# IST-DASLab/torch_cgx

Measured on AMD Instinct MI355X. Metric: DDP samples/sec ResNet-50 4-bit, higher is better.
Workload: dtype bf16; 1 GPU; model=resnet50, global_batch=256, input=3x224x224, parallelism=dp1, backend=cgx, bits=4, bucket_size=1024, compression_active=False

## Files before the change

csrc/bindings.cc:

```cpp
#include <torch/extension.h>

#include <ATen/hip/impl/HIPStreamMasqueradingAsCUDA.h>
#include <torch/csrc/utils/pybind.h>

#include <ATen/hip/impl/HIPGuardImplMasqueradingAsCUDA.h>

#include <cstring>
#include <functional>
#include <thread>
#include <tuple>

#include "backend.h"
#include "bn_plan.h"
#include "collectives.h"
#include "reducer.h"

namespace cgx {
namespace {

void run_rank_threads(int ws, int dev,
                      const std::function<void(int, hipStream_t)>& body,
                      const std::function<void()>& abort) {
  std::vector<hipStream_t> qs(ws, nullptr);
  for (auto& s : qs)
// ... 506 lines not shown
  if (!bn_tensor_ok(dy)) dy = dy.contiguous(at::MemoryFormat::ChannelsLast);
  if (!bn_tensor_ok(dy)) dy = dy.clone(at::MemoryFormat::ChannelsLast);
  if (mask.has_value())
    TORCH_CHECK(mask->is_cuda() && mask->scalar_type() == at::kByte &&
                    mask->is_contiguous() && mask->numel() == x.numel() / 8,
                "bn_act_backward: mask must hold one bit per element");
  auto dx = at::empty(x.sizes(), x.options(), at::MemoryFormat::ChannelsLast);
  auto stats = x.options().dtype(at::kFloat);
  auto dgamma = at::empty({c}, stats), dbeta = at::empty({c}, stats);
  c10::optional<at::Tensor> didentity;
  if (has_identity)
    didentity = mask.has_value()
                    ? at::empty(x.sizes(), x.options(),
                                at::MemoryFormat::ChannelsLast)
                    : dy;
  auto part = bn_workspace(p, x);
  BnBackwardArgs a;
  a.dy = dy.data_ptr();
  a.x = x.data_ptr();
  a.mean = bn_channel_vec(mean, c, "mean");
  a.invstd = bn_channel_vec(invstd, c, "invstd");
  a.weight = bn_channel_vec(weight, c, "weight");
  a.mask = mask.has_value() ? mask->data_ptr<uint8_t>() : nullptr;
  a.dx = dx.data_ptr();
  a.didentity =
      has_identity && mask.has_value() ? didentity->data_ptr() : nullptr;
  a.dgamma = dgamma.data_ptr<float>();
  a.dbeta = dbeta.data_ptr<float>();
  a.part = part.data_ptr<float>();
  launch_bn_backward(
      p, a, c10::hip::getCurrentHIPStreamMasqueradingAsCUDA(
                x.device().index()).stream());
  return {dx, dgamma, dbeta, didentity};
}

py::dict py_bn_plan(int64_t rows, int64_t channels) {
  const BnPlan p = bn_plan(rows, channels);
  py::dict d;
  d["eligible"] = p.eligible;
  d["threads"] = kBnThreads;
  d["cgs"] = p.cgs;
  d["tile_cgs"] = p.tc;
  d["ctiles"] = p.ctiles;
  d["rows_per_iter"] = p.rln;
  d["splits"] = p.splits;
  d["grid"] = p.grid;
  d["rows_per_thread"] = p.rows_per_thread;
  d["partial_floats"] = p.partial_floats;
  return d;
}

at::Tensor py_bn_sweep_indices(int64_t rows, int64_t channels) {
  const BnPlan p = bn_plan(rows, channels);
  TORCH_CHECK(p.eligible, "bn_sweep_indices: shape is not eligible");
  auto out = at::full({(int64_t)p.grid * kBnThreads, p.rows_per_thread + 1},
                      -1, at::TensorOptions().dtype(at::kLong));
  int64_t* o = out.data_ptr<int64_t>();
  const int64_t width = p.rows_per_thread + 1;
  for (int wg = 0; wg < p.grid; wg++)
    for (int tid = 0; tid < kBnThreads; tid++) {
      const BnSweep sw = bn_sweep(p, wg, tid);
      int64_t k = 0;
      for (int64_t r = sw.row; r < p.rows; r += sw.stride, k++) {
        TORCH_CHECK(k < width, "bn_sweep_indices: run longer than planned");
        o[((int64_t)wg * kBnThreads + tid) * width + k] = bn_vec(p, r, sw.cg);
      }
// ... 146 lines not shown
  m.def("plan_bucket", &cgx::py_plan_bucket, py::arg("layer_numels"),
        py::arg("layer_cfgs"), py::arg("dtype"), py::arg("fusion_bytes"),
        py::arg("min_elems"), py::arg("fake_ratio") = 1.0,
        py::arg("dummy") = false,
        "Test seam: the bucket plan for layers laid out back to back from "
        "byte offset 0 -> (uncomp [(byte_off, count)], chunks [[(byte_off, "
        "numel, bits, bucket)]]).");
  m.def("plan_chunk", &cgx::py_plan_chunk, py::arg("views"), py::arg("dtype"),
        py::arg("ws"), py::arg("skip_incomplete") = false,
        "Test seam: the rank plan of one chunk [(byte_off, numel, bits, "
        "bucket)] -> (offs, szs, comp, rs [[(byte_off, n, bits, bucket, "
        "comp_off, skip_incomplete, fb_off)]]).");
  m.def("route_quantize", &cgx::py_route_quantize, py::arg("slices"),
        "Test seam: the launch router's quantize plan for "
        "[(in, out, fb, n, bits, bucket, skip_incomplete)] (pointers as "
        "ints) -> [(bits, kind, descs, cum, any_residual, max_gpl)].");
  m.def("route_dequantize", &cgx::py_route_dequantize, py::arg("slices"),
        py::arg("dtype"), py::arg("src_stride") = 0, py::arg("nsrc") = 1,
        py::arg("add") = false,
        "Test seam: the launch router's dequantize plan for "
        "[(in, out, n, bits, bucket, skip_incomplete)] -> "
        "[(bits, kind, descs, total_groups, any_residual)].");
  m.def("bn_act_forward", &cgx::py_bn_act_forward, py::arg("x"),
        py::arg("identity"), py::arg("weight"), py::arg("bias"),
        py::arg("running_mean"), py::arg("running_var"), py::arg("momentum"),
        py::arg("eps"), py::arg("relu"),
        "Training-mode BatchNorm2d of a channels_last bf16 tensor, fused with "
        "an optional residual add and ReLU -> (out, mean, invstd, mask | "
        "None); updates the running statistics in place.");
  m.def("bn_act_backward", &cgx::py_bn_act_backward, py::arg("dy"),
        py::arg("x"), py::arg("mean"), py::arg("invstd"), py::arg("weight"),
        py::arg("mask"), py::arg("has_identity"),
        "Backward of bn_act_forward -> (dx, dgamma, dbeta, didentity | None).");
  m.def("bn_eligible", &cgx::py_bn_eligible, py::arg("x"),
        "True where the fused BatchNorm kernels take `x`: CUDA, bf16, dense "
        "channels_last, and a shape bn_plan calls eligible.");
  m.def("bn_plan", &cgx::py_bn_plan, py::arg("rows"), py::arg("channels"),
        "Test seam: the launch geometry of the fused BatchNorm kernels for a "
        "[rows, channels] activation.");
  m.def("bn_sweep_indices", &cgx::py_bn_sweep_indices, py::arg("rows"),
        py::arg("channels"),
        "Test seam: [grid*threads, rows_per_thread+1] int64, the 16-byte "
        "vector indices every thread visits (-1: none).");
  m.def("bn_partial_offsets", &cgx::py_bn_partial_offsets, py::arg("rows"),
        py::arg("channels"), py::arg("wg"),
        "Test seam: the partial-buffer floats workgroup `wg` writes.");
  m.attr("FLAG_SKIP_INCOMPLETE") = cgx::kFlagSkipIncomplete;
  m.attr("FLAG_TAIL_ONLY") = cgx::kFlagTailOnly;
  m.attr("KIND_FAST") = (int)cgx::kFast;
  m.attr("KIND_GENERIC") = (int)cgx::kGeneric;
  m.attr("KIND_TWO_PASS") = (int)cgx::kTwoPass;
  m.attr("KIND_SUB") = (int)cgx::kSub;
}
```

csrc/bn_kernels.hip:

```cpp
#include <hip/hip_runtime.h>

#include "bn_plan.h"
#include "check.h"

namespace cgx {
namespace {

constexpr int kT = kBnThreads;

__device__ inline void unpack8(const uint4& v, float (&f)[8]) {
  f[0] = __uint_as_float(v.x << 16);
  f[1] = __uint_as_float(v.x & 0xffff0000u);
  f[2] = __uint_as_float(v.y << 16);
  f[3] = __uint_as_float(v.y & 0xffff0000u);
  f[4] = __uint_as_float(v.z << 16);
  f[5] = __uint_as_float(v.z & 0xffff0000u);
  f[6] = __uint_as_float(v.w << 16);
  f[7] = __uint_as_float(v.w & 0xffff0000u);
}

__device__ inline unsigned bf16_bits(float f) {
  const unsigned u = __float_as_uint(f);
  if ((u & 0x7fffffffu) > 0x7f800000u) return (u >> 16) | 0x40u;
  return (u + 0x7fffu + ((u >> 16) & 1u)) >> 16;
// ... 351 lines not shown
    scale[j] *= invstd[j];
    mg[j] *= inv_r;
    mgx[j] *= inv_r;
  }
  auto one = [&](const uint4& dyv, const uint4& xv, unsigned mbits, int64_t i) {
    float g[8], xf[8];
    unsigned gb[8], o[8];
    masked_dy<RELU>(dyv, mbits, g, gb);
    unpack8(xv, xf);
#pragma unroll
    for (int j = 0; j < 8; j++) {
      const float xhat = (xf[j] - mean[j]) * invstd[j];
      o[j] = bf16_bits(scale[j] * ((g[j] - mg[j]) - xhat * mgx[j]));
    }
    dx[i] = pack8(o);
    if (ADD) didentity[i] = pack8(gb);
  };
  int64_t r = sw.row;
  for (; r + sw.stride < p.rows; r += 2 * sw.stride) {
    const int64_t i0 = bn_vec(p, r, sw.cg);
    const int64_t i1 = bn_vec(p, r + sw.stride, sw.cg);
    const uint4 a0 = dy[i0], a1 = dy[i1];
    const uint4 b0 = x[i0], b1 = x[i1];
    const unsigned m0 = RELU ? mask[i0] : 0xffu, m1 = RELU ? mask[i1] : 0xffu;
    one(a0, b0, m0, i0);
    one(a1, b1, m1, i1);
  }
  if (r < p.rows) {
    const int64_t i0 = bn_vec(p, r, sw.cg);
    one(dy[i0], x[i0], RELU ? mask[i0] : 0xffu, i0);
  }
}

int fin_grid(const BnPlan& p) {
  return (p.channels + kBnFinChannels - 1) / kBnFinChannels;
}

}

void launch_bn_forward(const BnPlan& p, const BnForwardArgs& a,
                       hipStream_t stream) {
  float* pmean = a.part;
  float* pm2 = a.part + p.partial_floats;
  float* pcnt = a.part + 2 * p.partial_floats;
  const uint4* x = static_cast<const uint4*>(a.x);
  const uint4* idn = static_cast<const uint4*>(a.identity);
  uint4* out = static_cast<uint4*>(a.out);
  const dim3 grid(p.grid), block(kT);
  hipLaunchKernelGGL(bn_stats, grid, block, 0, stream, x, pmean, pm2, pcnt, p);
  hipLaunchKernelGGL(bn_stats_finalize, dim3(fin_grid(p)), block, 0, stream,
                     pmean, pm2, pcnt, a.mean, a.invstd, a.running_mean,
                     a.running_var, a.momentum, a.eps, p);
#define CGX_BN_APPLY(RELU, ADD)                                              \
  hipLaunchKernelGGL((bn_apply<RELU, ADD>), grid, block, 0, stream, x, idn,  \
                     a.mean, a.invstd, a.weight, a.bias, out, a.mask, p)
  if (a.relu && idn) CGX_BN_APPLY(true, true);
  else if (a.relu) CGX_BN_APPLY(true, false);
  else if (idn) CGX_BN_APPLY(false, true);
  else CGX_BN_APPLY(false, false);
#undef CGX_BN_APPLY
  CGX_HIP_CHECK(hipGetLastError());
}

void launch_bn_backward(const BnPlan& p, const BnBackwardArgs& a,
                        hipStream_t stream) {
  float* psg = a.part;
  float* psgx = a.part + p.partial_floats;
  const uint4* dy = static_cast<const uint4*>(a.dy);
  const uint4* x = static_cast<const uint4*>(a.x);
  uint4* dx = static_cast<uint4*>(a.dx);
  uint4* did = static_cast<uint4*>(a.didentity);
  const dim3 grid(p.grid), block(kT);
  if (a.mask)
    hipLaunchKernelGGL(bn_bwd_reduce<true>, grid, block, 0, stream, dy, x,
                       a.mask, a.mean, a.invstd, psg, psgx, p);
  else
    hipLaunchKernelGGL(bn_bwd_reduce<false>, grid, block, 0, stream, dy, x,
                       a.mask, a.mean, a.invstd, psg, psgx, p);
  hipLaunchKernelGGL(bn_bwd_finalize, dim3(fin_grid(p)), block, 0, stream, psg,
                     psgx, a.dbeta, a.dgamma, p);
#define CGX_BN_DX(RELU, ADD)                                                 \
  hipLaunchKernelGGL((bn_bwd_dx<RELU, ADD>), grid, block, 0, stream, dy, x,  \
                     a.mask, a.mean, a.invstd, a.weight, a.dbeta, a.dgamma,  \
                     dx, did, p)
  if (a.mask && did) CGX_BN_DX(true, true);
  else if (a.mask) CGX_BN_DX(true, false);
  else CGX_BN_DX(false, false);
#undef CGX_BN_DX
  CGX_HIP_CHECK(hipGetLastError());
}

}
```

csrc/bn_plan.cc:

```cpp
#include "bn_plan.h"

#include <algorithm>

namespace cgx {

BnPlan bn_plan(int64_t rows, int64_t channels) {
  BnPlan p;
  p.rows = rows;
  p.channels = (int)std::min<int64_t>(std::max<int64_t>(channels, 0), 1 << 30);
  const bool pow2 = channels > 0 && (channels & (channels - 1)) == 0;
  p.eligible = pow2 && channels >= 8 && channels <= 2048 && rows >= 2 &&
               rows <= kBnMaxRows;
  if (!p.eligible) return p;

  p.cgs = p.channels / 8;
  p.tc = std::min(p.cgs, kBnMaxTileCgs);
  p.ctiles = p.cgs / p.tc;
  p.rln = kBnThreads / p.tc;
  const int64_t row_blocks = (rows + p.rln - 1) / p.rln;
  int64_t splits = std::min<int64_t>(row_blocks,
                                     std::max(1, kBnTargetWgs / p.ctiles));
  splits = std::min(splits, std::max<int64_t>(1, rows / 80));
  p.splits = (int)splits;
  p.grid = p.ctiles * p.splits;
  p.rows_per_thread = (int)((row_blocks + splits - 1) / splits);
  p.partial_floats = (int64_t)p.splits * p.channels;
  return p;
}

}
```

csrc/bn_plan.h:

```cpp
#pragma once

#include <hip/hip_runtime.h>

#include <cstdint>

namespace cgx {

constexpr int kBnThreads = 256;
constexpr int kBnTargetWgs = 1024;
constexpr int kBnMaxTileCgs = 32;
constexpr int kBnFinChannels = 4;

struct BnPlan {
  int64_t rows = 0;
  int channels = 0;
  bool eligible = false;
  int cgs = 0;
  int tc = 0;
  int ctiles = 0;
  int rln = 0;
  int splits = 0;
  int grid = 0;
  int rows_per_thread = 0;
  int64_t partial_floats = 0;
// ... 29 lines not shown
  const void* x;
  const void* identity;
  const float* weight;
  const float* bias;
  float* running_mean;
  float* running_var;
  float momentum, eps;
  bool relu;
  void* out;
  float* mean;
  float* invstd;
  uint8_t* mask;
  float* part;
};
void launch_bn_forward(const BnPlan& p, const BnForwardArgs& a,
                       hipStream_t stream);

struct BnBackwardArgs {
  const void* dy;
  const void* x;
  const float* mean;
  const float* invstd;
  const float* weight;
  const uint8_t* mask;
  void* dx;
  void* didentity;
  float* dgamma;
  float* dbeta;
  float* part;
};
void launch_bn_backward(const BnPlan& p, const BnBackwardArgs& a,
                        hipStream_t stream);

}
```

torch_cgx_amd/models/resnet.py:

```python

from __future__ import annotations

import torch
import torch.nn as nn

from ..ops.fused_bn import bn_act


class Bottleneck(nn.Module):
    expansion = 4

    def __init__(self, inplanes: int, planes: int, stride: int = 1,
                 downsample: nn.Module = None):
        super().__init__()
        self.conv1 = nn.Conv2d(inplanes, planes, 1, bias=False)
        self.bn1 = nn.BatchNorm2d(planes)
        self.conv2 = nn.Conv2d(planes, planes, 3, stride=stride, padding=1,
                               bias=False)
        self.bn2 = nn.BatchNorm2d(planes)
        self.conv3 = nn.Conv2d(planes, planes * self.expansion, 1, bias=False)
        self.bn3 = nn.BatchNorm2d(planes * self.expansion)
        self.relu = nn.ReLU(inplace=True)
        self.downsample = downsample
        self.stride = stride

    def forward(self, x):
        identity = x
        out = bn_act(self.bn1, self.conv1(x))
        out = bn_act(self.bn2, self.conv2(out))
        out = self.conv3(out)
        if self.downsample is not None:
            identity = self.downsample(x)
        return bn_act(self.bn3, out, identity)


class ResNet(nn.Module):
    def __init__(self, layers, num_classes: int = 1000):
        super().__init__()
        self.inplanes = 64
        self.conv1 = nn.Conv2d(3, 64, 7, stride=2, padding=3, bias=False)
        self.bn1 = nn.BatchNorm2d(64)
        self.relu = nn.ReLU(inplace=True)
        self.maxpool = nn.MaxPool2d(3, stride=2, padding=1)
        self.layer1 = self._make_layer(64, layers[0])
        self.layer2 = self._make_layer(128, layers[1], stride=2)
        self.layer3 = self._make_layer(256, layers[2], stride=2)
        self.layer4 = self._make_layer(512, layers[3], stride=2)
        self.avgpool = nn.AdaptiveAvgPool2d(1)
        self.fc = nn.Linear(512 * Bottleneck.expansion, num_classes)
        for m in self.modules():
            if isinstance(m, nn.Conv2d):
                nn.init.kaiming_normal_(m.weight, mode="fan_out",
                                        nonlinearity="relu")
            elif isinstance(m, nn.BatchNorm2d):
                nn.init.constant_(m.weight, 1)
                nn.init.constant_(m.bias, 0)

    def _make_layer(self, planes: int, blocks: int, stride: int = 1):
        downsample = None
        if stride != 1 or self.inplanes != planes * Bottleneck.expansion:
            downsample = nn.Sequential(
                nn.Conv2d(self.inplanes, planes * Bottleneck.expansion, 1,
                          stride=stride, bias=False),
                nn.BatchNorm2d(planes * Bottleneck.expansion),
            )
        layers = [Bottleneck(self.inplanes, planes, stride, downsample)]
        self.inplanes = planes * Bottleneck.expansion
        for _ in range(1, blocks):
            layers.append(Bottleneck(self.inplanes, planes))
        return nn.Sequential(*layers)

    def forward(self, x):
        x = self.maxpool(bn_act(self.bn1, self.conv1(x)))
        x = self.layer4(self.layer3(self.layer2(self.layer1(x))))
        x = self.avgpool(x).flatten(1)
        return self.fc(x)


def resnet50(num_classes: int = 1000) -> ResNet:
    return ResNet([3, 4, 6, 3], num_classes)


def resnet18(num_classes: int = 1000) -> nn.Module:

    class BasicBlock(nn.Module):
        def __init__(self, inp, planes, stride=1, down=None):
            super().__init__()
            self.c1 = nn.Conv2d(inp, planes, 3, stride, 1, bias=False)
            self.b1 = nn.BatchNorm2d(planes)
            self.c2 = nn.Conv2d(planes, planes, 3, 1, 1, bias=False)
            self.b2 = nn.BatchNorm2d(planes)
            self.down = down

        def forward(self, x):
            idt = x if self.down is None else self.down(x)
            out = torch.relu(self.b1(self.c1(x)))
            return torch.relu(self.b2(self.c2(out)) + idt)

    class R18(nn.Module):
        def __init__(self):
            super().__init__()
            self.stem = nn.Sequential(
                nn.Conv2d(3, 64, 7, 2, 3, bias=False), nn.BatchNorm2d(64),
                nn.ReLU(inplace=True), nn.MaxPool2d(3, 2, 1))
            chans = [64, 128, 256, 512]
            blocks = []
# ... 21 lines not shown
```

torch_cgx_amd/ops/fused_bn.py:

```python

from __future__ import annotations

import os

import torch
import torch.nn.functional as F

from .. import _C


class _BnAct(torch.autograd.Function):
    @staticmethod
    def forward(ctx, x, identity, weight, bias, running_mean, running_var,
                momentum, eps, relu):
        out, mean, invstd, mask = _C.bn_act_forward(
            x, identity, weight, bias, running_mean, running_var, momentum,
            eps, relu)
        ctx.save_for_backward(x, mean, invstd, weight, mask)
        ctx.has_identity = identity is not None
        return out

    @staticmethod
    def backward(ctx, dy):
        x, mean, invstd, weight, mask = ctx.saved_tensors
        dx, dgamma, dbeta, didentity = _C.bn_act_backward(
            dy, x, mean, invstd, weight, mask, ctx.has_identity)
        return (dx, didentity, dgamma, dbeta, None, None, None, None, None)


def fused_bn_enabled() -> bool:
    return os.environ.get("CGX_FUSED_BN", "1") != "0"


def _native(bn, x, identity) -> bool:
    if not (bn.training and bn.track_running_stats
            and bn.momentum is not None and fused_bn_enabled()):
        return False
    if bn.weight is None or bn.bias is None:
        return False
    if not (x.is_cuda and _C.bn_eligible(x)):
        return False
    if identity is not None and not (
            identity.shape == x.shape and identity.device == x.device
            and _C.bn_eligible(identity)):
        return False
    return bn.weight.dtype == torch.float32


def bn_act(bn: torch.nn.BatchNorm2d, x: torch.Tensor,
           identity: torch.Tensor = None, relu: bool = True) -> torch.Tensor:
    if _native(bn, x, identity):
        bn.num_batches_tracked.add_(1)
        return _BnAct.apply(x, identity, bn.weight, bn.bias, bn.running_mean,
                            bn.running_var, bn.momentum, bn.eps, relu)
    out = bn(x)
    if identity is not None:
        out = out + identity
    if relu:
        out = F.relu(out, inplace=True)
    return out
```

Measured before the change: 7077 samples/s.

## Fuse downsample BatchNorm into residual join and stem BN+ReLU into maxpool

```diff
diff --git a/csrc/bindings.cc b/csrc/bindings.cc
--- a/csrc/bindings.cc
+++ b/csrc/bindings.cc
@@ -562,6 +562,221 @@
       p, a, c10::hip::getCurrentHIPStreamMasqueradingAsCUDA(
                 x.device().index()).stream());
   return {dx, dgamma, dbeta, didentity};
+}
+
+hipStream_t bn_stream(const at::Tensor& x) {
+  return c10::hip::getCurrentHIPStreamMasqueradingAsCUDA(x.device().index())
+      .stream();
+}
+
+at::Tensor bn_dense_dy(at::Tensor dy) {
+  if (!bn_tensor_ok(dy)) dy = dy.contiguous(at::MemoryFormat::ChannelsLast);
+  if (!bn_tensor_ok(dy)) dy = dy.clone(at::MemoryFormat::ChannelsLast);
+  return dy;
+}
+
+std::tuple<at::Tensor, at::Tensor, at::Tensor, at::Tensor, at::Tensor,
+           c10::optional<at::Tensor>>
+py_bn_act2_forward(const at::Tensor& x3, const at::Tensor& xd,
+                   const at::Tensor& weight3, const at::Tensor& bias3,
+                   at::Tensor running_mean3, at::Tensor running_var3,
+                   double momentum3, double eps3, const at::Tensor& weightd,
+                   const at::Tensor& biasd, at::Tensor running_meand,
+                   at::Tensor running_vard, double momentumd, double epsd,
+                   bool relu) {
+  TORCH_CHECK(py_bn_eligible(x3), "bn_act2_forward: input is not eligible");
+  TORCH_CHECK(bn_tensor_ok(xd) && xd.sizes() == x3.sizes() &&
+                  xd.device() == x3.device(),
+              "bn_act2_forward: both inputs must have the same shape");
+  const BnPlan p = bn_plan_of(x3);
+  const int64_t c = p.channels;
+  c10::hip::HIPGuardMasqueradingAsCUDA guard(x3.device().index());
+  auto out = at::empty(x3.sizes(), x3.options(), at::MemoryFormat::ChannelsLast);
+  auto stats = x3.options().dtype(at::kFloat);
+  auto mean3 = at::empty({c}, stats), invstd3 = at::empty({c}, stats);
+  auto meand = at::empty({c}, stats), invstdd = at::empty({c}, stats);
+  c10::optional<at::Tensor> mask;
+  if (relu) mask = at::empty({x3.numel() / 8}, x3.options().dtype(at::kByte));
+  auto part = at::empty({2 * (2 * p.partial_floats + p.grid)}, stats);
+  BnJoinArgs j{};
+  j.a.x = x3.data_ptr();
+  j.a.weight = bn_channel_vec(weight3, c, "weight");
+  j.a.bias = bn_channel_vec(bias3, c, "bias");
+  j.a.running_mean = bn_channel_vec(running_mean3, c, "running_mean");
+  j.a.running_var = bn_channel_vec(running_var3, c, "running_var");
+  j.a.momentum = (float)momentum3;
+  j.a.eps = (float)eps3;
+  j.a.mean = mean3.data_ptr<float>();
+  j.a.invstd = invstd3.data_ptr<float>();
+  j.b.x = xd.data_ptr();
+  j.b.weight = bn_channel_vec(weightd, c, "identity weight");
+  j.b.bias = bn_channel_vec(biasd, c, "identity bias");
+  j.b.running_mean = bn_channel_vec(running_meand, c, "identity running_mean");
+  j.b.running_var = bn_channel_vec(running_vard, c, "identity running_var");
+  j.b.momentum = (float)momentumd;
+  j.b.eps = (float)epsd;
+  j.b.mean = meand.data_ptr<float>();
+  j.b.invstd = invstdd.data_ptr<float>();
+  j.relu = relu;
+  j.out = out.data_ptr();
+  j.mask = relu ? mask->data_ptr<uint8_t>() : nullptr;
+  j.part = part.data_ptr<float>();
+  launch_bn_join_forward(p, j, bn_stream(x3));
+  return {out, mean3, invstd3, meand, invstdd, mask};
+}
+
+std::tuple<at::Tensor, at::Tensor, at::Tensor, at::Tensor, at::Tensor,
+           at::Tensor>
+py_bn_act2_backward(at::Tensor dy, const at::Tensor& x3, const at::Tensor& xd,
+                    const at::Tensor& mean3, const at::Tensor& invstd3,
+                    const at::Tensor& weight3, const at::Tensor& meand,
+                    const at::Tensor& invstdd, const at::Tensor& weightd,
+                    const c10::optional<at::Tensor>& mask) {
+  TORCH_CHECK(py_bn_eligible(x3), "bn_act2_backward: input is not eligible");
+  TORCH_CHECK(bn_tensor_ok(xd) && xd.sizes() == x3.sizes() &&
+                  xd.device() == x3.device(),
+              "bn_act2_backward: both inputs must have the same shape");
+  const BnPlan p = bn_plan_of(x3);
+  const int64_t c = p.channels;
+  TORCH_CHECK(dy.is_cuda() && dy.device() == x3.device() &&
+                  dy.scalar_type() == at::kBFloat16 && dy.sizes() == x3.sizes(),
+              "bn_act2_backward: dy must match the input");
+  c10::hip::HIPGuardMasqueradingAsCUDA guard(x3.device().index());
+  dy = bn_dense_dy(dy);
+  if (mask.has_value())
+    TORCH_CHECK(mask->is_cuda() && mask->scalar_type() == at::kByte &&
+                    mask->is_contiguous() && mask->numel() == x3.numel() / 8,
+                "bn_act2_backward: mask must hold one bit per element");
+  auto dx3 = at::empty(x3.sizes(), x3.options(), at::MemoryFormat::ChannelsLast);
+  auto dxd = at::empty(x3.sizes(), x3.options(), at::MemoryFormat::ChannelsLast);
+  auto stats = x3.options().dtype(at::kFloat);
+  auto dgamma3 = at::empty({c}, stats), dbeta3 = at::empty({c}, stats);
+  auto dgammad = at::empty({c}, stats), dbetad = at::empty({c}, stats);
+  auto part = at::empty({3 * p.partial_floats}, stats);
+  BnJoinArgs j{};
+  j.a.x = x3.data_ptr();
+  j.a.mean = bn_channel_vec(mean3, c, "mean");
+  j.a.invstd = bn_channel_vec(invstd3, c, "invstd");
+  j.a.weight = bn_channel_vec(weight3, c, "weight");
+  j.a.dx = dx3.data_ptr();
+  j.a.dgamma = dgamma3.data_ptr<float>();
+  j.a.dbeta = dbeta3.data_ptr<float>();
+  j.b.x = xd.data_ptr();
+  j.b.mean = bn_channel_vec(meand, c, "identity mean");
+  j.b.invstd = bn_channel_vec(invstdd, c, "identity invstd");
+  j.b.weight = bn_channel_vec(weightd, c, "identity weight");
+  j.b.dx = dxd.data_ptr();
+  j.b.dgamma = dgammad.data_ptr<float>();
+  j.b.dbeta = dbetad.data_ptr<float>();
+  j.dy = dy.data_ptr();
+  j.mask = mask.has_value() ? mask->data_ptr<uint8_t>() : nullptr;
+  j.part = part.data_ptr<float>();
+  launch_bn_join_backward(p, j, bn_stream(x3));
+  return {dx3, dxd, dgamma3, dbeta3, dgammad, dbetad};
+}
+
+BnPoolPlan bn_pool_plan_of(const at::Tensor& x) {
+  return bn_pool_plan(x.size(0), x.size(2), x.size(3), x.size(1));
+}
+
+std::tuple<at::Tensor, at::Tensor, at::Tensor, at::Tensor>
+py_bn_act_pool_forward(const at::Tensor& x, const at::Tensor& weight,
+                       const at::Tensor& bias, at::Tensor running_mean,
+                       at::Tensor running_var, double momentum, double eps) {
+  TORCH_CHECK(py_bn_eligible(x), "bn_act_pool_forward: input is not eligible");
+  const BnPlan p = bn_plan_of(x);
+  const BnPoolPlan g = bn_pool_plan_of(x);
+  const int64_t c = p.channels;
+  c10::hip::HIPGuardMasqueradingAsCUDA guard(x.device().index());
+  auto out = at::empty({x.size(0), c, g.oh, g.ow}, x.options(),
+                       at::MemoryFormat::ChannelsLast);
+  auto arg = at::empty({x.size(0), c, g.oh, g.ow},
+                       x.options().dtype(at::kByte),
+                       at::MemoryFormat::ChannelsLast);
+  auto stats = x.options().dtype(at::kFloat);
+  auto mean = at::empty({c}, stats), invstd = at::empty({c}, stats);
+  auto part = bn_workspace(p, x);
+  BnPoolArgs a{};
+  a.x = x.data_ptr();
+  a.weight = bn_channel_vec(weight, c, "weight");
+  a.bias = bn_channel_vec(bias, c, "bias");
+  a.running_mean = bn_channel_vec(running_mean, c, "running_mean");
+  a.running_var = bn_channel_vec(running_var, c, "running_var");
+  a.momentum = (float)momentum;
+  a.eps = (float)eps;
+  a.mean = mean.data_ptr<float>();
+  a.invstd = invstd.data_ptr<float>();
+  a.out = out.data_ptr();
+  a.arg = arg.data_ptr<uint8_t>();
+  a.part = part.data_ptr<float>();
+  launch_bn_pool_forward(p, g, a, bn_stream(x));
+  return {out, mean, invstd, arg};
+}
+
+std::tuple<at::Tensor, at::Tensor, at::Tensor>
+py_bn_act_pool_backward(at::Tensor dy, const at::Tensor& x,
+                        const at::Tensor& mean, const at::Tensor& invstd,
+                        const at::Tensor& weight, const at::Tensor& arg) {
+  TORCH_CHECK(py_bn_eligible(x), "bn_act_pool_backward: input is not eligible");
+  const BnPlan p = bn_plan_of(x);
+  const BnPoolPlan g = bn_pool_plan_of(x);
+  const int64_t c = p.channels;
+  const std::vector<int64_t> pooled = {x.size(0), c, g.oh, g.ow};
+  TORCH_CHECK(dy.is_cuda() && dy.device() == x.device() &&
+                  dy.scalar_type() == at::kBFloat16 && dy.sizes() == at::IntArrayRef(pooled),
+              "bn_act_pool_backward: dy must have the pooled shape");
+  TORCH_CHECK(arg.is_cuda() && arg.device() == x.device() &&
+                  arg.scalar_type() == at::kByte && arg.sizes() == at::IntArrayRef(pooled) &&
+                  arg.is_contiguous(at::MemoryFormat::ChannelsLast) &&
+                  reinterpret_cast<uintptr_t>(arg.data_ptr()) % 8 == 0,
+              "bn_act_pool_backward: arg must be the forward's");
+  c10::hip::HIPGuardMasqueradingAsCUDA guard(x.device().index());
+  dy = bn_dense_dy(dy);
+  auto dx = at::empty(x.sizes(), x.options(), at::MemoryFormat::ChannelsLast);
+  auto stats = x.options().dtype(at::kFloat);
+  auto dgamma = at::empty({c}, stats), dbeta = at::empty({c}, stats);
+  auto part = bn_workspace(p, x);
+  BnPoolArgs a{};
+  a.x = x.data_ptr();
+  a.mean = bn_channel_vec(mean, c, "mean");
+  a.invstd = bn_channel_vec(invstd, c, "invstd");
+  a.weight = bn_channel_vec(weight, c, "weight");
+  a.arg = arg.data_ptr<uint8_t>();
+  a.dy = dy.data_ptr();
+  a.dx = dx.data_ptr();
+  a.dgamma = dgamma.data_ptr<float>();
+  a.dbeta = dbeta.data_ptr<float>();
+  a.part = part.data_ptr<float>();
+  launch_bn_pool_backward(p, g, a, bn_stream(x));
+  return {dx, dgamma, dbeta};
+}
+
+std::tuple<at::Tensor, at::Tensor> py_bn_pool_geometry(int64_t h, int64_t w) {
+  TORCH_CHECK(h >= 1 && w >= 1 && h * w <= kBnMaxRows, "bn_pool_geometry: bad");
+  const BnPoolPlan g = bn_pool_plan(1, h, w, 8);
+  auto opt = at::TensorOptions().dtype(at::kLong);
+  auto windows = at::full({(int64_t)g.oh * g.ow, 9}, -1, opt);
+  auto covers = at::full({h * w, 4, 2}, -1, opt);
+  int64_t* wi = windows.data_ptr<int64_t>();
+  int64_t* co = covers.data_ptr<int64_t>();
+  for (int oh = 0; oh < g.oh; oh++)
+    for (int ow = 0; ow < g.ow; ow++)
+      for (int k = 0; k < 9; k++) {
+        const int ih = pool_in(oh, k / 3), iw = pool_in(ow, k % 3);
+        if (ih >= 0 && ih < g.h && iw >= 0 && iw < g.w)
+          wi[((int64_t)oh * g.ow + ow) * 9 + k] = (int64_t)ih * g.w + iw;
+      }
+  for (int ih = 0; ih < g.h; ih++)
+    for (int iw = 0; iw < g.w; iw++) {
+      int n = 0;
+      for (int oh = pool_cover_lo(ih); oh <= pool_cover_hi(ih, g.oh); oh++)
+        for (int ow = pool_cover_lo(iw); ow <= pool_cover_hi(iw, g.ow); ow++) {
+          int64_t* e = co + (((int64_t)ih * g.w + iw) * 4 + n++) * 2;
+          e[0] = (int64_t)oh * g.ow + ow;
+          e[1] = pool_k(ih, oh) * 3 + pool_k(iw, ow);
+        }
+    }
+  return {windows, covers};
 }
 
 py::dict py_bn_plan(int64_t rows, int64_t channels) {
@@ -774,6 +989,28 @@
         py::arg("x"), py::arg("mean"), py::arg("invstd"), py::arg("weight"),
         py::arg("mask"), py::arg("has_identity"),
         "Backward of bn_act_forward -> (dx, dgamma, dbeta, didentity | None).");
+  m.def("bn_act2_forward", &cgx::py_bn_act2_forward,
+        "relu(bn3(x3) + bn_d(xd)) with both BatchNorms in training mode: "
+        "(x3, xd, weight3, bias3, running_mean3, running_var3, momentum3, "
+        "eps3, weightd, biasd, running_meand, running_vard, momentumd, epsd, "
+        "relu) -> (out, mean3, invstd3, meand, invstdd, mask | None).");
+  m.def("bn_act2_backward", &cgx::py_bn_act2_backward,
+        "Backward of bn_act2_forward: (dy, x3, xd, mean3, invstd3, weight3, "
+        "meand, invstdd, weightd, mask) -> (dx3, dxd, dgamma3, dbeta3, "
+        "dgammad, dbetad).");
+  m.def("bn_act_pool_forward", &cgx::py_bn_act_pool_forward, py::arg("x"),
+        py::arg("weight"), py::arg("bias"), py::arg("running_mean"),
+        py::arg("running_var"), py::arg("momentum"), py::arg("eps"),
+        "max_pool2d(relu(bn(x)), 3, 2, 1) in training mode -> (pooled, mean, "
+        "invstd, arg); arg is one byte per pooled element.");
+  m.def("bn_act_pool_backward", &cgx::py_bn_act_pool_backward, py::arg("dy"),
+        py::arg("x"), py::arg("mean"), py::arg("invstd"), py::arg("weight"),
+        py::arg("arg"),
+        "Backward of bn_act_pool_forward -> (dx, dgamma, dbeta).");
+  m.def("bn_pool_geometry", &cgx::py_bn_pool_geometry, py::arg("h"),
+        py::arg("w"),
+        "Test seam: (windows [oh*ow, 9], covers [h*w, 4, 2]) of the stem's "
+        "3x3/2/1 pooling as the kernels index it.");
   m.def("bn_eligible", &cgx::py_bn_eligible, py::arg("x"),
         "True where the fused BatchNorm kernels take `x`: CUDA, bf16, dense "
         "channels_last, and a shape bn_plan calls eligible.");
diff --git a/csrc/bn_kernels.hip b/csrc/bn_kernels.hip
--- a/csrc/bn_kernels.hip
+++ b/csrc/bn_kernels.hip
@@ -407,25 +407,375 @@
   }
 }
 
+
+struct Affine {
+  float mean[8], invstd[8], gamma[8], beta[8];
+  __device__ void load(const float* mean_, const float* invstd_,
+                       const float* weight, const float* bias, int cg) {
+    load_k(mean, mean_ + cg * 8);
+    load_k(invstd, invstd_ + cg * 8);
+    load_k(gamma, weight + cg * 8);
+    load_k(beta, bias + cg * 8);
+  }
+};
+
+template <bool RELU>
+__global__ __launch_bounds__(kT) void bn_apply_join(
+    const uint4* __restrict__ x3, const uint4* __restrict__ xd,
+    const float* __restrict__ mean3, const float* __restrict__ invstd3,
+    const float* __restrict__ weight3, const float* __restrict__ bias3,
+    const float* __restrict__ meand, const float* __restrict__ invstdd,
+    const float* __restrict__ weightd, const float* __restrict__ biasd,
+    uint4* __restrict__ out, uint8_t* __restrict__ mask, BnPlan p) {
+  const BnSweep sw = bn_sweep(p, blockIdx.x, threadIdx.x);
+  Affine a, b;
+  a.load(mean3, invstd3, weight3, bias3, sw.cg);
+  b.load(meand, invstdd, weightd, biasd, sw.cg);
+  auto one = [&](const uint4& xv, const uint4& dv, int64_t i) {
+    float d[8];
+    unsigned idb[8];
+    unpack8(dv, d);
+#pragma unroll
+    for (int j = 0; j < 8; j++)
+      idb[j] = bf16_bits(((d[j] - b.mean[j]) * b.invstd[j]) * b.gamma[j] +
+                         b.beta[j]);
+    apply_one<RELU, true>(xv, pack8(idb), a.mean, a.invstd, a.gamma, a.beta,
+                          out, mask, i);
+  };
+  int64_t r = sw.row;
+  for (; r + sw.stride < p.rows; r += 2 * sw.stride) {
+    const int64_t i0 = bn_vec(p, r, sw.cg);
+    const int64_t i1 = bn_vec(p, r + sw.stride, sw.cg);
+    const uint4 a0 = x3[i0], a1 = x3[i1];
+    const uint4 d0 = xd[i0], d1 = xd[i1];
+    one(a0, d0, i0);
+    one(a1, d1, i1);
+  }
+  if (r < p.rows) {
+    const int64_t i0 = bn_vec(p, r, sw.cg);
+    one(x3[i0], xd[i0], i0);
+  }
+}
+
+template <bool RELU>
+__global__ __launch_bounds__(kT) void bn_bwd_reduce_join(
+    const uint4* __restrict__ dy, const uint4* __restrict__ x3,
+    const uint4* __restrict__ xd, const uint8_t* __restrict__ mask,
+    const float* __restrict__ mean3_, const float* __restrict__ invstd3_,
+    const float* __restrict__ meand_, const float* __restrict__ invstdd_,
+    float* __restrict__ psg, float* __restrict__ psgx3,
+    float* __restrict__ psgxd, BnPlan p) {
+  __shared__ float sh[24][kT];
+  const int tid = threadIdx.x;
+  const BnSweep sw = bn_sweep(p, blockIdx.x, tid);
+  float mean3[8], invstd3[8], meand[8], invstdd[8];
+  load_k(mean3, mean3_ + sw.cg * 8);
+  load_k(invstd3, invstd3_ + sw.cg * 8);
+  load_k(meand, meand_ + sw.cg * 8);
+  load_k(invstdd, invstdd_ + sw.cg * 8);
+  float s[24] = {};
+  auto accumulate = [&](const uint4& dyv, const uint4& av, const uint4& bv,
+                        unsigned mbits) {
+    float g[8], af[8], bf[8];
+    unsigned gb[8];
+    masked_dy<RELU>(dyv, mbits, g, gb);
+    unpack8(av, af);
+    unpack8(bv, bf);
+#pragma unroll
+    for (int j = 0; j < 8; j++) {
+      const float xhat3 = (af[j] - mean3[j]) * invstd3[j];
+      const float xhatd = (bf[j] - meand[j]) * invstdd[j];
+      s[j] += g[j];
+      s[8 + j] = fmaf(g[j], xhat3, s[8 + j]);
+      s[16 + j] = fmaf(g[j], xhatd, s[16 + j]);
+    }
+  };
+  int64_t r = sw.row;
+  for (; r + sw.stride < p.rows; r += 2 * sw.stride) {
+    const int64_t i0 = bn_vec(p, r, sw.cg);
+    const int64_t i1 = bn_vec(p, r + sw.stride, sw.cg);
+    const uint4 a0 = dy[i0], a1 = dy[i1];
+    const uint4 b0 = x3[i0], b1 = x3[i1];
+    const uint4 c0 = xd[i0], c1 = xd[i1];
+    const unsigned m0 = RELU ? mask[i0] : 0xffu, m1 = RELU ? mask[i1] : 0xffu;
+    accumulate(a0, b0, c0, m0);
+    accumulate(a1, b1, c1, m1);
+  }
+  if (r < p.rows) {
+    const int64_t i0 = bn_vec(p, r, sw.cg);
+    accumulate(dy[i0], x3[i0], xd[i0], RELU ? mask[i0] : 0xffu);
+  }
+  wg_sum<24>(s, sh, tid, p.tc);
+  if (tid < p.tc) {
+    const int64_t o = bn_partial_offset(p, blockIdx.x, sw.cg);
+#pragma unroll
+    for (int j = 0; j < 8; j++) {
+      psg[o + j] = s[j];
+      psgx3[o + j] = s[8 + j];
+      psgxd[o + j] = s[16 + j];
+    }
+  }
+}
+
+template <bool RELU>
+__global__ __launch_bounds__(kT) void bn_bwd_dx_join(
+    const uint4* __restrict__ dy, const uint4* __restrict__ x3,
+    const uint4* __restrict__ xd, const uint8_t* __restrict__ mask,
+    const float* __restrict__ mean3_, const float* __restrict__ invstd3_,
+    const float* __restrict__ weight3, const float* __restrict__ dgamma3,
+    const float* __restrict__ meand_, const float* __restrict__ invstdd_,
+    const float* __restrict__ weightd, const float* __restrict__ dgammad,
+    const float* __restrict__ dbeta, uint4* __restrict__ dx3,
+    uint4* __restrict__ dxd, BnPlan p) {
+  const BnSweep sw = bn_sweep(p, blockIdx.x, threadIdx.x);
+  float mean3[8], invstd3[8], scale3[8], mgx3[8];
+  float meand[8], invstdd[8], scaled[8], mgxd[8], mg[8];
+  load_k(mean3, mean3_ + sw.cg * 8);
+  load_k(invstd3, invstd3_ + sw.cg * 8);
+  load_k(scale3, weight3 + sw.cg * 8);
+  load_k(mgx3, dgamma3 + sw.cg * 8);
+  load_k(meand, meand_ + sw.cg * 8);
+  load_k(invstdd, invstdd_ + sw.cg * 8);
+  load_k(scaled, weightd + sw.cg * 8);
+  load_k(mgxd, dgammad + sw.cg * 8);
+  load_k(mg, dbeta + sw.cg * 8);
+  const float inv_r = 1.f / (float)p.rows;
+#pragma unroll
+  for (int j = 0; j < 8; j++) {
+    scale3[j] *= invstd3[j];
+    scaled[j] *= invstdd[j];
+    mg[j] *= inv_r;
+    mgx3[j] *= inv_r;
+    mgxd[j] *= inv_r;
+  }
+  auto one = [&](const uint4& dyv, const uint4& av, const uint4& bv,
+                 unsigned mbits, int64_t i) {
+    float g[8], af[8], bf[8];
+    unsigned gb[8], o3[8], od[8];
+    masked_dy<RELU>(dyv, mbits, g, gb);
+    unpack8(av, af);
+    unpack8(bv, bf);
+#pragma unroll
+    for (int j = 0; j < 8; j++) {
+      const float xhat3 = (af[j] - mean3[j]) * invstd3[j];
+      const float xhatd = (bf[j] - meand[j]) * invstdd[j];
+      o3[j] = bf16_bits(scale3[j] * ((g[j] - mg[j]) - xhat3 * mgx3[j]));
+      od[j] = bf16_bits(scaled[j] * ((g[j] - mg[j]) - xhatd * mgxd[j]));
+    }
+    dx3[i] = pack8(o3);
+    dxd[i] = pack8(od);
+  };
+  int64_t r = sw.row;
+  for (; r + sw.stride < p.rows; r += 2 * sw.stride) {
+    const int64_t i0 = bn_vec(p, r, sw.cg);
+    const int64_t i1 = bn_vec(p, r + sw.stride, sw.cg);
+    const uint4 a0 = dy[i0], a1 = dy[i1];
+    const uint4 b0 = x3[i0], b1 = x3[i1];
+    const uint4 c0 = xd[i0], c1 = xd[i1];
+    const unsigned m0 = RELU ? mask[i0] : 0xffu, m1 = RELU ? mask[i1] : 0xffu;
+    one(a0, b0, c0, m0, i0);
+    one(a1, b1, c1, m1, i1);
+  }
+  if (r < p.rows) {
+    const int64_t i0 = bn_vec(p, r, sw.cg);
+    one(dy[i0], x3[i0], xd[i0], RELU ? mask[i0] : 0xffu, i0);
+  }
+}
+
+
+__global__ __launch_bounds__(kT) void bn_apply_pool(
+    const uint4* __restrict__ x, const float* __restrict__ mean_,
+    const float* __restrict__ invstd_, const float* __restrict__ weight,
+    const float* __restrict__ bias, uint4* __restrict__ out,
+    uint2* __restrict__ arg, BnPoolPlan g) {
+  const int64_t t = (int64_t)blockIdx.x * kT + threadIdx.x;
+  if (t >= g.threads) return;
+  const int cg = (int)(t % g.cgs);
+  int pix = (int)(t / g.cgs);
+  const int ow = pix % g.ow;
+  pix /= g.ow;
+  const int oh = pix % g.oh, n = pix / g.oh;
+  float mean[8], invstd[8], gamma[8], beta[8];
+  load_k(mean, mean_ + cg * 8);
+  load_k(invstd, invstd_ + cg * 8);
+  load_k(gamma, weight + cg * 8);
+  load_k(beta, bias + cg * 8);
+  uint4 v[9];
+  bool live[9];
+#pragma unroll
+  for (int k = 0; k < 9; k++) {
+    const int ih = pool_in(oh, k / 3), iw = pool_in(ow, k % 3);
+    live[k] = ih >= 0 && ih < g.h && iw >= 0 && iw < g.w;
+    v[k] = live[k] ? x[(((int64_t)n * g.h + ih) * g.w + iw) * g.cgs + cg]
+                   : make_uint4(0, 0, 0, 0);
+  }
+  float best[8];
+  unsigned bits[8], pos[8];
+#pragma unroll
+  for (int j = 0; j < 8; j++) {
+    best[j] = -INFINITY;
+    bits[j] = 0;
+    pos[j] = kPoolNone;
+  }
+#pragma unroll
+  for (int k = 0; k < 9; k++) {
+    if (!live[k]) continue;
+    float f[8];
+    unpack8(v[k], f);
+#pragma unroll
+    for (int j = 0; j < 8; j++) {
+      const float y = ((f[j] - mean[j]) * invstd[j]) * gamma[j] + beta[j];
+      unsigned b = bf16_bits(y);
+      float z = __uint_as_float(b << 16);
+      if (z <= 0.f) {
+        b = 0;
+        z = 0.f;
+      }
+      if (z > best[j] || z != z) {
+        best[j] = z;
+        bits[j] = b;
+        pos[j] = k;
+      }
+    }
+  }
+#pragma unroll
+  for (int j = 0; j < 8; j++)
+    if (best[j] <= 0.f) pos[j] = kPoolNone;
+  out[t] = pack8(bits);
+  arg[t] = make_uint2(pos[0] | (pos[1] << 8) | (pos[2] << 16) | (pos[3] << 24),
+                      pos[4] | (pos[5] << 8) | (pos[6] << 16) | (pos[7] << 24));
+}
+
+__device__ inline void pooled_g(const uint4* __restrict__ dy,
+                                const uint2* __restrict__ arg,
+                                const BnPoolPlan& pl, int64_t row, int cg,
+                                float (&g)[8]) {
+  int pix = (int)row;
+  const int iw = pix % pl.w;
+  pix /= pl.w;
+  const int ih = pix % pl.h, n = pix / pl.h;
+  const int oh0 = pool_cover_lo(ih), oh1 = pool_cover_hi(ih, pl.oh);
+  const int ow0 = pool_cover_lo(iw), ow1 = pool_cover_hi(iw, pl.ow);
+  float acc[8] = {};
+  for (int oh = oh0; oh <= oh1; oh++)
+    for (int ow = ow0; ow <= ow1; ow++) {
+      const int64_t i = (((int64_t)n * pl.oh + oh) * pl.ow + ow) * pl.cgs + cg;
+      const unsigned k = pool_k(ih, oh) * 3 + pool_k(iw, ow);
+      const uint4 dv = dy[i];
+      const uint2 av = arg[i];
+      float d[8];
+      unpack8(dv, d);
+#pragma unroll
+      for (int j = 0; j < 8; j++) {
+        const unsigned a = ((j < 4 ? av.x : av.y) >> (8 * (j & 3))) & 0xffu;
+        if (a == k) acc[j] += d[j];
+      }
+    }
+#pragma unroll
+  for (int j = 0; j < 8; j++) g[j] = __uint_as_float(bf16_bits(acc[j]) << 16);
+}
+
+__global__ __launch_bounds__(kT) void bn_pool_bwd_reduce(
+    const uint4* __restrict__ dy, const uint2* __restrict__ arg,
+    const uint4* __restrict__ x, const float* __restrict__ mean_,
+    const float* __restrict__ invstd_, float* __restrict__ psg,
+    float* __restrict__ psgx, BnPlan p, BnPoolPlan pl) {
+  __shared__ float sh[16][kT];
+  const int tid = threadIdx.x;
+  const BnSweep sw = bn_sweep(p, blockIdx.x, tid);
+  float mean[8], invstd[8];
+  load_k(mean, mean_ + sw.cg * 8);
+  load_k(invstd, invstd_ + sw.cg * 8);
+  float s[16] = {};
+#pragma unroll 2
+  for (int64_t r = sw.row; r < p.rows; r += sw.stride) {
+    const uint4 xv = x[bn_vec(p, r, sw.cg)];
+    float g[8], xf[8];
+    pooled_g(dy, arg, pl, r, sw.cg, g);
+    unpack8(xv, xf);
+#pragma unroll
+    for (int j = 0; j < 8; j++) {
+      const float xhat = (xf[j] - mean[j]) * invstd[j];
+      s[j] += g[j];
+      s[8 + j] = fmaf(g[j], xhat, s[8 + j]);
+    }
+  }
+  wg_sum<16>(s, sh, tid, p.tc);
+  if (tid < p.tc) {
+    const int64_t o = bn_partial_offset(p, blockIdx.x, sw.cg);
+#pragma unroll
+    for (int j = 0; j < 8; j++) {
+      psg[o + j] = s[j];
+      psgx[o + j] = s[8 + j];
+    }
+  }
+}
+
+__global__ __launch_bounds__(kT) void bn_pool_bwd_dx(
+    const uint4* __restrict__ dy, const uint2* __restrict__ arg,
+    const uint4* __restrict__ x, const float* __restrict__ mean_,
+    const float* __restrict__ invstd_, const float* __restrict__ weight,
+    const float* __restrict__ dbeta, const float* __restrict__ dgamma,
+    uint4* __restrict__ dx, BnPlan p, BnPoolPlan pl) {
+  const BnSweep sw = bn_sweep(p, blockIdx.x, threadIdx.x);
+  float mean[8], invstd[8], scale[8], mg[8], mgx[8];
+  load_k(mean, mean_ + sw.cg * 8);
+  load_k(invstd, invstd_ + sw.cg * 8);
+  load_k(scale, weight + sw.cg * 8);
+  load_k(mg, dbeta + sw.cg * 8);
+  load_k(mgx, dgamma + sw.cg * 8);
+  const float inv_r = 1.f / (float)p.rows;
+#pragma unroll
+  for (int j = 0; j < 8; j++) {
+    scale[j] *= invstd[j];
+    mg[j] *= inv_r;
+    mgx[j] *= inv_r;
+  }
+#pragma unroll 2
+  for (int64_t r = sw.row; r < p.rows; r += sw.stride) {
+    const int64_t i = bn_vec(p, r, sw.cg);
+    const uint4 xv = x[i];
+    float g[8], xf[8];
+    unsigned o[8];
+    pooled_g(dy, arg, pl, r, sw.cg, g);
+    unpack8(xv, xf);
+#pragma unroll
+    for (int j = 0; j < 8; j++) {
+      const float xhat = (xf[j] - mean[j]) * invstd[j];
+      o[j] = bf16_bits(scale[j] * ((g[j] - mg[j]) - xhat * mgx[j]));
+    }
+    dx[i] = pack8(o);
+  }
+}
+
 int fin_grid(const BnPlan& p) {
   return (p.channels + kBnFinChannels - 1) / kBnFinChannels;
 }
 
+void launch_bn_stats(const BnPlan& p, const void* x_, float* part, float* mean,
+                     float* invstd, float* running_mean, float* running_var,
+                     float momentum, float eps, hipStream_t stream) {
+  float* pmean = part;
+  float* pm2 = part + p.partial_floats;
+  float* pcnt = part + 2 * p.partial_floats;
+  const uint4* x = static_cast<const uint4*>(x_);
+  hipLaunchKernelGGL(bn_stats, dim3(p.grid), dim3(kT), 0, stream, x, pmean,
+                     pm2, pcnt, p);
+  hipLaunchKernelGGL(bn_stats_finalize, dim3(fin_grid(p)), dim3(kT), 0, stream,
+                     pmean, pm2, pcnt, mean, invstd, running_mean, running_var,
+                     momentum, eps, p);
+}
+
 }
 
 void launch_bn_forward(const BnPlan& p, const BnForwardArgs& a,
                        hipStream_t stream) {
-  float* pmean = a.part;
-  float* pm2 = a.part + p.partial_floats;
-  float* pcnt = a.part + 2 * p.partial_floats;
   const uint4* x = static_cast<const uint4*>(a.x);
   const uint4* idn = static_cast<const uint4*>(a.identity);
   uint4* out = static_cast<uint4*>(a.out);
   const dim3 grid(p.grid), block(kT);
-  hipLaunchKernelGGL(bn_stats, grid, block, 0, stream, x, pmean, pm2, pcnt, p);
-  hipLaunchKernelGGL(bn_stats_finalize, dim3(fin_grid(p)), block, 0, stream,
-                     pmean, pm2, pcnt, a.mean, a.invstd, a.running_mean,
-                     a.running_var, a.momentum, a.eps, p);
+  launch_bn_stats(p, a.x, a.part, a.mean, a.invstd, a.running_mean,
+                  a.running_var, a.momentum, a.eps, stream);
 #define CGX_BN_APPLY(RELU, ADD)                                              \
   hipLaunchKernelGGL((bn_apply<RELU, ADD>), grid, block, 0, stream, x, idn,  \
                      a.mean, a.invstd, a.weight, a.bias, out, a.mask, p)
@@ -465,4 +815,91 @@
   CGX_HIP_CHECK(hipGetLastError());
 }
 
-}
+void launch_bn_join_forward(const BnPlan& p, const BnJoinArgs& j,
+                            hipStream_t stream) {
+  const BnOperand &a = j.a, &b = j.b;
+  float* part_b = j.part + 2 * p.partial_floats + p.grid;
+  launch_bn_stats(p, a.x, j.part, a.mean, a.invstd, a.running_mean,
+                  a.running_var, a.momentum, a.eps, stream);
+  launch_bn_stats(p, b.x, part_b, b.mean, b.invstd, b.running_mean,
+                  b.running_var, b.momentum, b.eps, stream);
+  const uint4* x3 = static_cast<const uint4*>(a.x);
+  const uint4* xd = static_cast<const uint4*>(b.x);
+  uint4* out = static_cast<uint4*>(j.out);
+  const dim3 grid(p.grid), block(kT);
+  if (j.relu)
+    hipLaunchKernelGGL(bn_apply_join<true>, grid, block, 0, stream, x3, xd,
+                       a.mean, a.invstd, a.weight, a.bias, b.mean, b.invstd,
+                       b.weight, b.bias, out, j.mask, p);
+  else
+    hipLaunchKernelGGL(bn_apply_join<false>, grid, block, 0, stream, x3, xd,
+                       a.mean, a.invstd, a.weight, a.bias, b.mean, b.invstd,
+                       b.weight, b.bias, out, j.mask, p);
+  CGX_HIP_CHECK(hipGetLastError());
+}
+
+void launch_bn_join_backward(const BnPlan& p, const BnJoinArgs& j,
+                             hipStream_t stream) {
+  const BnOperand &a = j.a, &b = j.b;
+  float* psg = j.part;
+  float* psgx3 = j.part + p.partial_floats;
+  float* psgxd = j.part + 2 * p.partial_floats;
+  const uint4* dy = static_cast<const uint4*>(j.dy);
+  const uint4* x3 = static_cast<const uint4*>(a.x);
+  const uint4* xd = static_cast<const uint4*>(b.x);
+  uint4* dx3 = static_cast<uint4*>(a.dx);
+  uint4* dxd = static_cast<uint4*>(b.dx);
+  const dim3 grid(p.grid), block(kT), fin(fin_grid(p));
+  if (j.mask)
+    hipLaunchKernelGGL(bn_bwd_reduce_join<true>, grid, block, 0, stream, dy, x3,
+                       xd, j.mask, a.mean, a.invstd, b.mean, b.invstd, psg,
+                       psgx3, psgxd, p);
+  else
+    hipLaunchKernelGGL(bn_bwd_reduce_join<false>, grid, block, 0, stream, dy,
+                       x3, xd, j.mask, a.mean, a.invstd, b.mean, b.invstd, psg,
+                       psgx3, psgxd, p);
+  hipLaunchKernelGGL(bn_bwd_finalize, fin, block, 0, stream, psg, psgx3,
+                     a.dbeta, a.dgamma, p);
+  hipLaunchKernelGGL(bn_bwd_finalize, fin, block, 0, stream, psg, psgxd,
+                     b.dbeta, b.dgamma, p);
+  if (j.mask)
+    hipLaunchKernelGGL(bn_bwd_dx_join<true>, grid, block, 0, stream, dy, x3, xd,
+                       j.mask, a.mean, a.invstd, a.weight, a.dgamma, b.mean,
+                       b.invstd, b.weight, b.dgamma, a.dbeta, dx3, dxd, p);
+  else
+    hipLaunchKernelGGL(bn_bwd_dx_join<false>, grid, block, 0, stream, dy, x3,
+                       xd, j.mask, a.mean, a.invstd, a.weight, a.dgamma, b.mean,
+                       b.invstd, b.weight, b.dgamma, a.dbeta, dx3, dxd, p);
+  CGX_HIP_CHECK(hipGetLastError());
+}
+
+void launch_bn_pool_forward(const BnPlan& p, const BnPoolPlan& g,
+                            const BnPoolArgs& a, hipStream_t stream) {
+  launch_bn_stats(p, a.x, a.part, a.mean, a.invstd, a.running_mean,
+                  a.running_var, a.momentum, a.eps, stream);
+  hipLaunchKernelGGL(bn_apply_pool, dim3(g.grid), dim3(kT), 0, stream,
+                     static_cast<const uint4*>(a.x), a.mean, a.invstd, a.weight,
+                     a.bias, static_cast<uint4*>(a.out),
+                     reinterpret_cast<uint2*>(a.arg), g);
+  CGX_HIP_CHECK(hipGetLastError());
+}
+
+void launch_bn_pool_backward(const BnPlan& p, const BnPoolPlan& g,
+                             const BnPoolArgs& a, hipStream_t stream) {
+  float* psg = a.part;
+  float* psgx = a.part + p.partial_floats;
+  const uint4* dy = static_cast<const uint4*>(a.dy);
+  const uint2* arg = reinterpret_cast<const uint2*>(a.arg);
+  const uint4* x = static_cast<const uint4*>(a.x);
+  const dim3 grid(p.grid), block(kT);
+  hipLaunchKernelGGL(bn_pool_bwd_reduce, grid, block, 0, stream, dy, arg, x,
+                     a.mean, a.invstd, psg, psgx, p, g);
+  hipLaunchKernelGGL(bn_bwd_finalize, dim3(fin_grid(p)), block, 0, stream, psg,
+                     psgx, a.dbeta, a.dgamma, p);
+  hipLaunchKernelGGL(bn_pool_bwd_dx, grid, block, 0, stream, dy, arg, x, a.mean,
+                     a.invstd, a.weight, a.dbeta, a.dgamma,
+                     static_cast<uint4*>(a.dx), p, g);
+  CGX_HIP_CHECK(hipGetLastError());
+}
+
+}
diff --git a/csrc/bn_plan.cc b/csrc/bn_plan.cc
--- a/csrc/bn_plan.cc
+++ b/csrc/bn_plan.cc
@@ -28,4 +28,17 @@
   return p;
 }
 
+BnPoolPlan bn_pool_plan(int64_t n, int64_t h, int64_t w, int64_t channels) {
+  BnPoolPlan g;
+  g.n = (int)n;
+  g.h = (int)h;
+  g.w = (int)w;
+  g.oh = pool_out(g.h);
+  g.ow = pool_out(g.w);
+  g.cgs = (int)(channels / 8);
+  g.threads = (int64_t)g.n * g.oh * g.ow * g.cgs;
+  g.grid = (int)((g.threads + kBnThreads - 1) / kBnThreads);
+  return g;
 }
+
+}
diff --git a/csrc/bn_plan.h b/csrc/bn_plan.h
--- a/csrc/bn_plan.h
+++ b/csrc/bn_plan.h
@@ -85,4 +85,72 @@
 void launch_bn_backward(const BnPlan& p, const BnBackwardArgs& a,
                         hipStream_t stream);
 
+struct BnOperand {
+  const void* x;
+  const float* weight;
+  const float* bias;
+  float* running_mean;
+  float* running_var;
+  float momentum, eps;
+  float* mean;
+  float* invstd;
+  void* dx;
+  float* dgamma;
+  float* dbeta;
+};
+struct BnJoinArgs {
+  BnOperand a, b;
+  bool relu;
+  void* out;
+  const void* dy;
+  uint8_t* mask;
+  float* part;
+};
+void launch_bn_join_forward(const BnPlan& p, const BnJoinArgs& a,
+                            hipStream_t stream);
+void launch_bn_join_backward(const BnPlan& p, const BnJoinArgs& a,
+                             hipStream_t stream);
+
+constexpr int kPoolNone = 9;
+
+struct BnPoolPlan {
+  int n = 0, h = 0, w = 0;
+  int oh = 0, ow = 0;
+  int cgs = 0;
+  int64_t threads = 0;
+  int grid = 0;
+};
+BnPoolPlan bn_pool_plan(int64_t n, int64_t h, int64_t w, int64_t channels);
+
+__host__ __device__ inline int pool_out(int in) { return (in - 1) / 2 + 1; }
+__host__ __device__ inline int pool_in(int o, int k) { return 2 * o - 1 + k; }
+__host__ __device__ inline int pool_cover_lo(int i) { return i / 2; }
+__host__ __device__ inline int pool_cover_hi(int i, int out) {
+  const int hi = (i + 1) / 2;
+  return hi < out ? hi : out - 1;
 }
+__host__ __device__ inline int pool_k(int i, int o) { return i - (2 * o - 1); }
+
+struct BnPoolArgs {
+  const void* x;
+  const float* weight;
+  const float* bias;
+  float* running_mean;
+  float* running_var;
+  float momentum, eps;
+  float* mean;
+  float* invstd;
+  void* out;
+  uint8_t* arg;
+  const void* dy;
+  void* dx;
+  float* dgamma;
+  float* dbeta;
+  float* part;
+};
+void launch_bn_pool_forward(const BnPlan& p, const BnPoolPlan& g,
+                            const BnPoolArgs& a, hipStream_t stream);
+void launch_bn_pool_backward(const BnPlan& p, const BnPoolPlan& g,
+                             const BnPoolArgs& a, hipStream_t stream);
+
+}
diff --git a/torch_cgx_amd/models/resnet.py b/torch_cgx_amd/models/resnet.py
--- a/torch_cgx_amd/models/resnet.py
+++ b/torch_cgx_amd/models/resnet.py
@@ -4,7 +4,7 @@
 import torch
 import torch.nn as nn
 
-from ..ops.fused_bn import bn_act
+from ..ops.fused_bn import bn_act, bn_act_pool
 
 
 class Bottleneck(nn.Module):
@@ -30,7 +30,8 @@
         out = bn_act(self.bn2, self.conv2(out))
         out = self.conv3(out)
         if self.downsample is not None:
-            identity = self.downsample(x)
+            conv, bn = self.downsample[0], self.downsample[1]
+            return bn_act(self.bn3, out, conv(x), identity_bn=bn)
         return bn_act(self.bn3, out, identity)
 
 
@@ -71,7 +72,7 @@
         return nn.Sequential(*layers)
 
     def forward(self, x):
-        x = self.maxpool(bn_act(self.bn1, self.conv1(x)))
+        x = bn_act_pool(self.bn1, self.conv1(x), self.maxpool)
         x = self.layer4(self.layer3(self.layer2(self.layer1(x))))
         x = self.avgpool(x).flatten(1)
         return self.fc(x)
diff --git a/torch_cgx_amd/ops/fused_bn.py b/torch_cgx_amd/ops/fused_bn.py
--- a/torch_cgx_amd/ops/fused_bn.py
+++ b/torch_cgx_amd/ops/fused_bn.py
@@ -28,6 +28,45 @@
         return (dx, didentity, dgamma, dbeta, None, None, None, None, None)
 
 
+class _BnActJoin(torch.autograd.Function):
+    @staticmethod
+    def forward(ctx, x, xd, weight, bias, running_mean, running_var, momentum,
+                eps, weightd, biasd, running_meand, running_vard, momentumd,
+                epsd, relu):
+        out, mean, invstd, meand, invstdd, mask = _C.bn_act2_forward(
+            x, xd, weight, bias, running_mean, running_var, momentum, eps,
+            weightd, biasd, running_meand, running_vard, momentumd, epsd, relu)
+        ctx.save_for_backward(x, xd, mean, invstd, weight, meand, invstdd,
+                              weightd, mask)
+        return out
+
+    @staticmethod
+    def backward(ctx, dy):
+        (x, xd, mean, invstd, weight, meand, invstdd, weightd,
+         mask) = ctx.saved_tensors
+        dx, dxd, dgamma, dbeta, dgammad, dbetad = _C.bn_act2_backward(
+            dy, x, xd, mean, invstd, weight, meand, invstdd, weightd, mask)
+        return (dx, dxd, dgamma, dbeta, None, None, None, None, dgammad,
+                dbetad, None, None, None, None, None)
+
+
+class _BnActPool(torch.autograd.Function):
+    @staticmethod
+    def forward(ctx, x, weight, bias, running_mean, running_var, momentum,
+                eps):
+        out, mean, invstd, arg = _C.bn_act_pool_forward(
+            x, weight, bias, running_mean, running_var, momentum, eps)
+        ctx.save_for_backward(x, mean, invstd, weight, arg)
+        return out
+
+    @staticmethod
+    def backward(ctx, dy):
+        x, mean, invstd, weight, arg = ctx.saved_tensors
+        dx, dgamma, dbeta = _C.bn_act_pool_backward(dy, x, mean, invstd,
+                                                    weight, arg)
+        return (dx, dgamma, dbeta, None, None, None, None)
+
+
 def fused_bn_enabled() -> bool:
     return os.environ.get("CGX_FUSED_BN", "1") != "0"
 
@@ -47,15 +86,46 @@
     return bn.weight.dtype == torch.float32
 
 
+def _bn_args(bn):
+    return (bn.weight, bn.bias, bn.running_mean, bn.running_var, bn.momentum,
+            bn.eps)
+
+
 def bn_act(bn: torch.nn.BatchNorm2d, x: torch.Tensor,
-           identity: torch.Tensor = None, relu: bool = True) -> torch.Tensor:
+           identity: torch.Tensor = None, relu: bool = True,
+           identity_bn: torch.nn.BatchNorm2d = None) -> torch.Tensor:
+    if identity_bn is not None:
+        if _native(bn, x, identity) and _native(identity_bn, identity, x):
+            bn.num_batches_tracked.add_(1)
+            identity_bn.num_batches_tracked.add_(1)
+            return _BnActJoin.apply(x, identity, *_bn_args(bn),
+                                    *_bn_args(identity_bn), relu)
+        out = bn(x) + identity_bn(identity)
+        return F.relu(out, inplace=True) if relu else out
     if _native(bn, x, identity):
         bn.num_batches_tracked.add_(1)
-        return _BnAct.apply(x, identity, bn.weight, bn.bias, bn.running_mean,
-                            bn.running_var, bn.momentum, bn.eps, relu)
+        return _BnAct.apply(x, identity, *_bn_args(bn), relu)
     out = bn(x)
     if identity is not None:
         out = out + identity
     if relu:
         out = F.relu(out, inplace=True)
     return out
+
+
+def _pool_is_3x3_s2_p1(pool) -> bool:
+    def pair(v):
+        return tuple(v) if isinstance(v, (tuple, list)) else (v, v)
+
+    return (type(pool) is torch.nn.MaxPool2d
+            and pair(pool.kernel_size) == (3, 3) and pair(pool.stride) == (2, 2)
+            and pair(pool.padding) == (1, 1) and pair(pool.dilation) == (1, 1)
+            and not pool.ceil_mode and not pool.return_indices)
+
+
+def bn_act_pool(bn: torch.nn.BatchNorm2d, x: torch.Tensor,
+                pool: torch.nn.Module) -> torch.Tensor:
+    if _pool_is_3x3_s2_p1(pool) and _native(bn, x, None):
+        bn.num_batches_tracked.add_(1)
+        return _BnActPool.apply(x, *_bn_args(bn))
+    return pool(bn_act(bn, x))
```

Measured after the change: 7426 samples/s (median of 6 runs). 1.05x the previous value.
